# geobacter-rs/rav1e

Measured on AMD Instinct MI355X. Metric: encoded frames/sec + Mpixels/sec, 4K 8-bit speed=10, 1/2/4/8 GPU vs host CPU, higher is better.
Workload: dtype u8

## Files before the change

rav1e_amd/csrc/rv_quant.h:

```cpp
#pragma once

#include "rv_device.h"
#include "rv_quant_tables.h"
#include "rv_rate_table.h"

namespace rv {

struct QCtx {
  int log_tx_scale;
  int32_t dc_quant, dc_offset, ac_quant, ac_offset0, ac_offset1, deadzone;
  uint32_t dc_a, dc_b, dc_s, ac_a, ac_b, ac_s;
};

__host__ __device__ __forceinline__ int q_log_tx_scale(int area) {
  return (area > 256) + (area > 1024);
}

__device__ __forceinline__ int q_lookup(int ac, int qindex, int delta_q, int bd) {
  int i = qindex + delta_q;
  i = i < 0 ? 0 : i > 255 ? 255 : i;
  return RV_QLOOKUP[(3 * ac + (bd - 8) / 2) * 256 + i];
}

__device__ __forceinline__ void q_divu_gen(uint32_t d, uint32_t &a, uint32_t &b, uint32_t &s) {
// ... 98 lines not shown
      q = q_divu(wadd(v, q_signum(v) * c.dc_offset), c.dc_a, c.dc_b, c.dc_s);
    } else if (i <= eob) {
      const int32_t a = v < 0 ? -v : v;
      const int32_t o = v > 0 && a >= (mode ? acq : acq2) ? c.ac_offset1 : c.ac_offset0;
      q = q_divu(wadd(v, q_signum(v) * o), c.ac_a, c.ac_b, c.ac_s);
      mode = (mode != 0 && q == 0) ? 0 : (q > 1 ? 1 : mode);
    } else {
      q = 0;
    }
    const int32_t r = wadd(wmul(q, i == 0 ? c.dc_quant : c.ac_quant), (q >> 31) & roff) >> s;
    put(scan[i], q, r);
  }
  return eob;
}

__device__ __forceinline__ int32_t q_dequant(const QCtx &c, int32_t q, int i) {
  return wadd(wmul(q, i == 0 ? c.dc_quant : c.ac_quant), (q >> 31) & ((1 << c.log_tx_scale) - 1)) >>
         c.log_tx_scale;
}

__device__ __forceinline__ uint64_t q_estimate_rate(int qindex, int tx_size, uint64_t fd) {
  const uint32_t *row =
      RV_RDO_RATE_TABLE + ((qindex / RV_RDO_QUANT_DIV) * 19 + tx_size) * RV_RDO_NUM_BINS;
  uint64_t down = fd / RV_RATE_EST_BIN_SIZE;
  down = down < RV_RDO_NUM_BINS - 2 ? down : RV_RDO_NUM_BINS - 2;
  const uint64_t up = down + 1;
  const int64_t x0 = (int64_t)(down * RV_RATE_EST_BIN_SIZE);
  const int64_t y0 = row[down], y1 = row[up];
  const int64_t slope = (int64_t)((uint64_t)(y1 - y0) << 8) / RV_RATE_EST_BIN_SIZE;
  const int64_t r = y0 + ((int64_t)((uint64_t)((int64_t)fd - x0) * (uint64_t)slope) >> 8);
// ... 5 lines not shown
```

rav1e_amd/csrc/rv_rdo.h:

```cpp
#pragma once

#include "rv_chain.h"
#include "rv_device.h"
#include "rv_quant.h"

namespace rv {

struct RdoPlane {
  rv_plane org;
  rv_plane ref[2];
  rv_plane dst;
  int32_t *levels;
  uint64_t *out;
  QCtx q;
};

struct RdoWinner {
  int32_t c;
  int32_t skip;
  double cost;
  uint64_t dist;
};

struct RdoArgs {
// ... 25 lines not shown

int rv_quant_ctx(int qindex, int tx_area, int is_intra, int bit_depth, int dc_delta_q,
                 int ac_delta_q, rv::QCtx *out);

int rv_rdo_candidates(const rv::RdoArgs &luma, const rv::RdoArgs &chroma, int hbd,
                      hipStream_t s, bool compound = false);

int rv_rdo_blocks2(const rv::RdoArgs &l, const rv::RdoArgs &c, int nl, int nc, int hbd,
                   hipStream_t s, int mode);
int rv_rdo_blocks(const rv::RdoArgs &a, bool luma, int nplanes, int n_tx_size, int hbd,
                  hipStream_t s, int mode);

int rv_rdo_args_put(const rv::RdoArgs *h, int n, rv::RdoArgs *dev, hipStream_t s);
int rv_rdo_candidates_list(const rv::RdoArgs *h, const rv::RdoArgs *dev, int nsets, int mode_a,
                           int hbd, hipStream_t s, int max_grid = 0, uint32_t *kp_cnt = nullptr,
                           unsigned long long *kp_t = nullptr);

int rv_rdo_intra(const rv::RdoArgs &luma, const rv::RdoArgs &chroma, int hbd, hipStream_t s);
```

rav1e_amd/csrc/rv_rdo.hip:

```cpp
#include <stdio.h>
#include <stdlib.h>
#include <string.h>

#include <type_traits>

#include "rv_intra.h"
#include "rv_rdo.h"
#include "rv_tx.h"

namespace rv {


__constant__ int8_t kRdoReg[2][16][8] = {
    {{0, 0, 0, 127, 0, 0, 0, 0}, {0, 2, -6, 126, 8, -2, 0, 0},
     {0, 2, -10, 122, 18, -4, 0, 0}, {0, 2, -12, 116, 28, -8, 2, 0},
     {0, 2, -14, 110, 38, -10, 2, 0}, {0, 2, -14, 102, 48, -12, 2, 0},
     {0, 2, -16, 94, 58, -12, 2, 0}, {0, 2, -14, 84, 66, -12, 2, 0},
     {0, 2, -14, 76, 76, -14, 2, 0}, {0, 2, -12, 66, 84, -14, 2, 0},
     {0, 2, -12, 58, 94, -16, 2, 0}, {0, 2, -12, 48, 102, -14, 2, 0},
     {0, 2, -10, 38, 110, -14, 2, 0}, {0, 2, -8, 28, 116, -12, 2, 0},
     {0, 0, -4, 18, 122, -10, 2, 0}, {0, 0, -2, 8, 126, -6, 2, 0}},
    {{0, 0, 0, 127, 0, 0, 0, 0}, {0, 0, -4, 126, 8, -2, 0, 0},
     {0, 0, -8, 122, 18, -4, 0, 0}, {0, 0, -10, 116, 28, -6, 0, 0},
     {0, 0, -12, 110, 38, -8, 0, 0}, {0, 0, -12, 102, 48, -10, 0, 0},
// ... 248 lines not shown
#pragma unroll 1
    for (int r0 = 0; r0 < RB; r0 += U) {
#pragma unroll
      for (int u = 0; u < U; u++) {
        const int r = r0 + u;
        g0[(u + 6) & 7] = mc_h<Px>(f0, w0 + (r + 6) * (P / 4), col, ib);
        g1[(u + 6) & 7] = mc_h<Px>(f1, w1 + (r + 6) * (P / 4), col, ib);
        const int32_t t = mc_prep_v(f0, g0, u, ib) + mc_prep_v(f1, g1, u, ib);
        pred[(band * RB + r) * N + col] = (Px)clamp_med3(round_shift(t, ib + 1), 0, maxv);
      }
    }
  }
  wave_sync();
}

__device__ __forceinline__ double rdo_bias(const RdoArgs &a, int mi_x, int mi_y, int m = 2) {
  if (!a.imp) return 0.65;
  const int x2 = mi_x + m < a.w_in_b ? mi_x + m : a.w_in_b;
  const int y2 = mi_y + m < a.h_in_b ? mi_y + m : a.h_in_b;
  float tot = 0.f;
  for (int y = mi_y; y < y2; y++)
    for (int x = mi_x; x < x2; x++) tot = __fadd_rn(tot, a.imp[(y >> 1) * a.w_imp + (x >> 1)]);
  return (double)__fdiv_rn(__fdiv_rn(tot, (float)(m * m)), 3.0f) + 0.65;
}
__device__ __forceinline__ uint64_t rdo_biased(uint64_t v, double bias) {
  return (uint64_t)((double)v * bias);
}

__device__ __forceinline__ uint64_t rdo_cdef_finish(int32_t ss, int32_t sd, uint32_t ss2,
                                                    uint32_t sd2, uint32_t ssd, int bd);
// ... 347 lines not shown
#pragma unroll 8
    for (int i = lane; i < N * DPR; i += LPB) {
      const int r = i / DPR, c = (i - r * DPR) * PPD;
      uint32_t v;
      __builtin_memcpy(&v, pred + r * N + c, 4);
      if (valid) __builtin_memcpy(dp + r * ds + c * B, &v, 4);
    }
    return;
  }
  const uint64_t d = group_sum<LPB>(rdo_dist_biased<Px, N, LPB, LUMA>(a, jb, o, ost, pred));
  if (valid && lane == 0) pl.out[(int64_t)jb.oi * 3 + 1] = d;
}

__host__ __device__ constexpr int cmax(int a, int b) { return a > b ? a : b; }

template <typename Px, typename Mid, int NPART>
struct LumaLds {
  static constexpr int kWinP = sizeof(Px) == 1 ? 80 : 144;
  static constexpr int kWinRows = 64 / NPART + 7;
  static constexpr int kCompRows = sizeof(Px) == 1 ? 16 : 8;
  static constexpr int kScr =
      cmax(cmax(cmax(kWinRows * kWinP, 16 * 65 * 4), 32 * 66 * (int)sizeof(Mid)),
           2 * (kCompRows + 7) * kWinP);
  static constexpr int kSlot = (kScr + 64 * 64 * (int)sizeof(Px) + 15) / 16 * 16;
};


template <typename Px>
__device__ __forceinline__ uint64_t luma_dist(const RdoArgs &a, const RdoJob &j, const Px *o,
                                              int64_t os, const Px *pred) {
  const int lane = rv_tid() & 63, by = lane >> 3, bx = lane & 7;
  const uint64_t v =
      rdo_cdef_8x8<Px>(o + (int64_t)(by * 8) * os + bx * 8, os, pred + by * 8 * 64 + bx * 8, 64, a.bd);
  const int px = j.bx + bx * 8, py = j.by + by * 8;
  return group_sum<64>(rdo_biased(v, rdo_bias(a, px >> 2, py >> 2)));
}

template <typename Px, int NPART, int MODE>
__device__ __forceinline__ void luma_front(const RdoArgs &a, const RdoPlane &pl, int t,
                                           const RdoJob &jb, bool valid, uint8_t *scr, Px *pred,
                                           bool skip_dist = true) {
  constexpr int N = 64, B = (int)sizeof(Px);
  constexpr int P = LumaLds<Px, int16_t, NPART>::kWinP;
  constexpr int RP = N / NPART;
  static_assert(RP % 8 == 0, "MC rows run in groups of 8");
  const int lane = rv_tid() & 63;
  const rv_plane &ref = pl.ref[jb.ref];
  const int ox = 0, oy = 0;
  const int bd = a.bd, ib = bd == 12 ? 2 : 4, maxv = (1 << bd) - 1;

  if constexpr (MODE == 3) {
    intra_fill<Px, 64, 64>(jb, reinterpret_cast<int32_t *>(scr), pred, bd, lane);
  } else if (MODE == 1 || (MODE == 2 && jb.comp)) {
    mc_compound<Px, 64, LumaLds<Px, int16_t, NPART>::kCompRows>(
        a, pl, jb, reinterpret_cast<uint32_t *>(scr), pred);
  } else
  {
    uint32_t *win = reinterpret_cast<uint32_t *>(scr);
// ... 79 lines not shown
          if (rf) {
            int32_t s = 0;
#pragma unroll
            for (int k = 1; k < 7; k++) s += __mul24(yt[k], ring[(u + k) & 7]);
            v = round_shift(s, vshift);
          } else {
            v = cf ? round_shift(ring[(u + 3) & 7], ib) : ring[(u + 3) & 7];
          }
          pred[(RP * half + r) * N + col] = (Px)clamp_med3(v, 0, maxv);
        }
      }
    }
    wave_sync();
  }

  const Px *o = plane_ptr<Px>(pl.org, jb.bx, jb.by);
  if (!a.commit && skip_dist) {
    const uint64_t d = luma_dist<Px>(a, jb, o, pl.org.stride, pred);
    if (valid && lane == 0) pl.out[(int64_t)jb.oi * 3 + 0] = d;
  }
  int s0, s1, s2;
  fwd_shifts<N>((bd - 8) / 2, s0, s1, s2);
  int32_t *fmid = reinterpret_cast<int32_t *>(scr);
  {
    int32_t v[N];
#pragma unroll
    for (int r = 0; r < N; r++) {
      const int16_t d = (int16_t)((int16_t)o[(int64_t)r * pl.org.stride + lane] -
                                  (int16_t)pred[r * N + lane]);
      v[r] = rdo_rsa((int32_t)d, -s0);
    }
    tx::fwd1d<1, N>(v, v);
#pragma unroll
    for (int r = 0; r < 16; r++) fmid[r * 65 + lane] = rdo_rsa(v[r], -s1);
  }
// ... 46 lines not shown
  const int32_t *src = fmid + (rr >> 1) * 65 + (rr & 1) * 32;
#pragma unroll
  for (int c = 0; c < 32; c++) {
    const int32_t x = src[c];
    if (pk) pk[c] = x;
    v[c] = tx::clampv(x, range);
  }
#pragma unroll
  for (int c = 32; c < 64; c++) v[c] = 0;
}
template <typename Mid>
__device__ __forceinline__ void luma_inv_row_tx(int32_t *v, Mid *dst, int range, int crange) {
  tx::inv1d<1, 64>(v, range);
#pragma unroll
  for (int c = 0; c < 64; c++) dst[c] = (Mid)tx::clampv(round_shift(v[c], 2), crange);
}

template <typename Px, typename Mid>
__device__ __forceinline__ void luma_back(const RdoArgs &a, const RdoPlane &pl, int t,
                                          const RdoJob &jb, bool valid, const Mid *imid,
                                          Px *pred) {
  constexpr int N = 64, B = (int)sizeof(Px);
  const int lane = rv_tid() & 63;
  const int bd = a.bd, maxv = (1 << bd) - 1;
  const int crange = bd + 6 > 16 ? bd + 6 : 16;
  {
    int32_t v[N];
#pragma unroll
    for (int r = 0; r < N; r++) v[r] = r < 32 ? (int32_t)imid[r * 66 + lane] : 0;
    tx::inv1d<1, N>(v, crange);
// ... 86 lines not shown
  if (b < luma.n_tx && b >= rdo_ntx(luma)) return;
  if (b < luma.n_tx)
    rdo_luma_body<Px, Mid, 2, MODE>(luma, luma.p[0], b, lds,
                              reinterpret_cast<Px *>(lds + L::kScr), scan);
  else
    rdo_chroma_pair<Px, MODE>(chroma, b - luma.n_tx, reinterpret_cast<int32_t *>(lds),
                        reinterpret_cast<Px *>(lds + 2 * 32 * 33 * 4), scan);
}

template <typename Px>
struct QuadLds {
  using L = LumaLds<Px, int16_t, sizeof(Px) == 1 ? 2 : 4>;
  static constexpr int kBytes = cmax(4 * L::kSlot, 3 * kChromaPair(sizeof(Px)));
};

#ifndef RV_RDO_PHASES
#define RV_RDO_PHASES 0
#endif
__device__ unsigned long long g_rdo_ph[3][8];
struct QuadPh {
  unsigned long long t[5];
};

template <typename Px, int MODE>
__device__ __forceinline__ void rdo_quad_luma(const RdoArgs &luma, int b, int n, int var,
                                              uint8_t *lds, const uint16_t *scan,
                                              QuadPh *ph = nullptr) {
  using L = typename QuadLds<Px>::L;
  constexpr int NPART = sizeof(Px) == 1 ? 2 : 4;
  const int wave = __builtin_amdgcn_readfirstlane(rv_tid() >> 6), lane = rv_tid() & 63;
  auto slot = [&](int q) __attribute__((always_inline)) { return lds + q * L::kSlot; };
  auto fmid = [&](int q) __attribute__((always_inline)) {
    return reinterpret_cast<int32_t *>(slot(q));
  };
  auto imid = [&](int q) __attribute__((always_inline)) {
    return reinterpret_cast<int16_t *>(slot(q));
  };
  auto pred = [&](int q) __attribute__((always_inline)) {
    return reinterpret_cast<Px *>(slot(q) + L::kScr);
  };
  const int t0 = 4 * b, t = t0 + wave;
  if (t0 >= n) return;
  const bool valid = t < n;
  RdoJob jb;
  if constexpr (MODE == 3)
    jb = rdo_job_intra<Px, 64>(luma, 0, valid ? t : n - 1);
  else
    jb = rdo_job<64>(luma, luma.p[0], valid ? t : n - 1);
  const bool late_dist = (var & 1) && !luma.commit;
  const bool prio = (var & 2) != 0;
  if (valid)
    luma_front<Px, NPART, MODE>(luma, luma.p[0], t, jb, true, slot(wave), pred(wave), !late_dist);
  __syncthreads();
  if (RV_RDO_PHASES && ph) ph->t[1] = wall_clock64();
  if (wave == 0) {
    if (prio) __builtin_amdgcn_s_setprio(2);
    const int q = lane >> 4;
    if (t0 + q < n) luma_fwd_row(fmid(q) + (lane & 15) * 65, luma.bd);
    if (prio) __builtin_amdgcn_s_setprio(0);
  } else if (late_dist && valid) {
    const uint64_t d = luma_dist<Px>(luma, jb, plane_ptr<Px>(luma.p[0].org, jb.bx, jb.by),
                                     luma.p[0].org.stride, pred(wave));
    if (lane == 0) luma.p[0].out[(int64_t)jb.oi * 3 + 0] = d;
  }
  __syncthreads();
  if (RV_RDO_PHASES && ph) ph->t[2] = wall_clock64();
  if (valid) luma_quantize(luma, luma.p[0], t, jb, true, fmid(wave), scan);
// ... 12 lines not shown
  } else if (wave == 2 && late_dist) {
    RdoJob j0;
    if constexpr (MODE == 3)
      j0 = rdo_job_intra<Px, 64>(luma, 0, t0);
    else
      j0 = rdo_job<64>(luma, luma.p[0], t0);
    const uint64_t d = luma_dist<Px>(luma, j0, plane_ptr<Px>(luma.p[0].org, j0.bx, j0.by),
                                     luma.p[0].org.stride, pred(0));
    if (lane == 0) luma.p[0].out[(int64_t)j0.oi * 3 + 0] = d;
  }
  __syncthreads();
  if (RV_RDO_PHASES && ph) ph->t[4] = wall_clock64();
  if (valid) luma_back<Px, int16_t>(luma, luma.p[0], t, jb, true, imid(wave), pred(wave));
}

template <typename Px, int MODE>
__device__ __forceinline__ void rdo_quad_chroma(const RdoArgs &chroma, int c, int pairs,
                                                uint8_t *lds, const uint16_t *scan) {
  const int wave = __builtin_amdgcn_readfirstlane(rv_tid() >> 6);
  const int pair = 3 * c + wave;
  if (wave == 3 || pair >= 2 * pairs) return;
  uint8_t *w = lds + wave * kChromaPair(sizeof(Px));
  rdo_chroma_pair<Px, MODE>(chroma, pair, reinterpret_cast<int32_t *>(w),
                            reinterpret_cast<Px *>(w + 2 * 32 * 33 * 4), scan, pairs);
}

template <typename Px, int MODE>
__device__ __forceinline__ void rdo_quad_chroma4(const RdoArgs &chroma, int c, int n, uint8_t *lds,
                                                 const uint16_t *scan) {
  constexpr int kSlab = rdo_slab_bytes<Px, 32>();
// ... 43 lines not shown
  __shared__ uint16_t scan[1024];
  if (kp_t && threadIdx.x == 0) atomicMin(kp_t, (unsigned long long)wall_clock64());
  const RdoArgs &la = A[0], &ca = A[1], &lb = A[2], &cb = A[3];
  const int na = rdo_ntx(la), ma = rdo_ntx(ca);
  const int nb = nsets > 1 ? rdo_ntx(lb) : 0, mb = nsets > 1 ? rdo_ntx(cb) : 0;
  if (kp_cnt && blockIdx.x == 0 && threadIdx.x == 0) {
    atomicAdd(kp_cnt + (MA ? 1 : 0), (uint32_t)na);
    atomicAdd(kp_cnt + (MA ? 3 : 2), (uint32_t)ma);
    if (nsets > 1) {
      atomicAdd(kp_cnt + (MB ? 1 : 0), (uint32_t)nb);
      atomicAdd(kp_cnt + (MB ? 3 : 2), (uint32_t)mb);
    }
  }
  const int pa = (ma + 1) / 2, pb = (mb + 1) / 2;
  const bool c4 = (var & 32) != 0;
  const int e0 = (na + 3) / 4, e1 = e0 + (c4 ? (2 * ma + 3) / 4 : (2 * pa + 2) / 3);
  const int e2 = e1 + (nb + 3) / 4, e3 = e2 + (c4 ? (2 * mb + 3) / 4 : (2 * pb + 2) / 3);
  const bool phd = RV_RDO_PHASES && (var & 16) && rv_tid() == 0;
  for (int b = blockIdx.x; b < e3; b += gridDim.x) {
    QuadPh ph;
    ph.t[0] = phd ? wall_clock64() : 0;
    QuadPh *pp = phd ? &ph : nullptr;
    int set = 2;
    if (b < e0) {
      stage_scan(scan, la.q_tx_index);
      rdo_quad_luma<Px, MA>(la, b, na, var, lds, scan, pp);
      set = MA;
    } else if (b < e1) {
      stage_scan(scan, ca.q_tx_index);
      if (c4)
        rdo_quad_chroma4<Px, MA>(ca, b - e0, ma, lds, scan);
      else
        rdo_quad_chroma<Px, MA>(ca, b - e0, pa, lds, scan);
    } else if (b < e2) {
      stage_scan(scan, lb.q_tx_index);
      rdo_quad_luma<Px, MB>(lb, b - e1, nb, var, lds, scan, pp);
      set = MB;
    } else {
      stage_scan(scan, cb.q_tx_index);
      if (c4)
        rdo_quad_chroma4<Px, MB>(cb, b - e2, mb, lds, scan);
      else
        rdo_quad_chroma<Px, MB>(cb, b - e2, pb, lds, scan);
    }
    __syncthreads();
    if (phd) {
      const unsigned long long te = wall_clock64();
      if (set < 2) {
        for (int k = 0; k < 4; k++) atomicAdd(&g_rdo_ph[set][k], ph.t[k + 1] - ph.t[k]);
        atomicAdd(&g_rdo_ph[set][4], te - ph.t[4]);
      } else {
        atomicAdd(&g_rdo_ph[2][0], te - ph.t[0]);
      }
      atomicAdd(&g_rdo_ph[set][5], 1ull);
    }
  }
  if (kp_t && threadIdx.x == 0) atomicMax(kp_t + 1, (unsigned long long)wall_clock64());
}

__global__ __launch_bounds__(256) void rdo_args_store_kernel(RdoArgs a0, RdoArgs a1, RdoArgs a2,
                                                              RdoArgs a3, int n, RdoArgs *out) {
  static_assert(sizeof(RdoArgs) % 4 == 0, "word copy");
  constexpr int W = (int)(sizeof(RdoArgs) / 4);
  for (int i = threadIdx.x; i < n * W; i += blockDim.x) {
    const int k = i / W, w = i - k * W;
// ... 129 lines not shown
  else
    rdo_launch<0>(luma, chroma, hbd, s, cpairs);
  RV_HIP_CHECK_LAUNCH();
  return RV_OK;
}

int rv_rdo_args_put(const RdoArgs *h, int n, RdoArgs *dev, hipStream_t s) {
  if (!h || !dev || n < 1 || n > 4) return rv_set_error(RV_EINVAL, "rv_rdo_args_put: bad arguments");
  rdo_args_store_kernel<<<1, 256, 0, s>>>(h[0], h[n > 1 ? 1 : 0], h[n > 2 ? 2 : 0], h[n > 3 ? 3 : 0],
                                          n, dev);
  RV_HIP_CHECK_LAUNCH();
  return RV_OK;
}

int rv_rdo_candidates_list(const RdoArgs *h, const RdoArgs *dev, int nsets, int mode_a, int hbd,
                           hipStream_t s, int max_grid, uint32_t *kp_cnt, unsigned long long *kp_t) {
  if (!h || !dev || nsets < 1 || nsets > 2 || mode_a < 0 || mode_a > 1 || (nsets == 2 && mode_a) ||
      h[0].commit || h[0].bd == 12)
    return rv_set_error(RV_EINVAL, "rv_rdo_candidates_list: bad arguments");
  for (int k = 0; k < 2 * nsets; k++)
    if (!h[k].list || !h[k].count)
      return rv_set_error(RV_EINVAL, "rv_rdo_candidates_list: the sets must be list-driven");
  static const bool phases = getenv("RAV1E_HIP_RDO_PHASES") && getenv("RAV1E_HIP_RDO_PHASES")[0] == '1';
  const int var = kRdoVariant | (phases && max_grid > 0 ? 16 : 0) | (max_grid > 0 ? 32 : 0);
  unsigned full = 0;
  for (int k = 0; k < nsets; k++)
    full += (unsigned)((h[2 * k].n_tx + 3) / 4) +
            ((var & 32) ? (unsigned)(2 * h[2 * k + 1].n_tx + 3) / 4
                        : (unsigned)(2 * ((h[2 * k + 1].n_tx + 1) / 2) + 2) / 3);
  unsigned grid = std::min(full, kF4Pool);
  if (max_grid > 0) grid = std::min(grid, (unsigned)max_grid);
  if (grid == 0) return RV_OK;
#define RV_LIST(PX, MA, MB) \
  rdo_quad_list_kernel<PX, MA, MB><<<grid, 256, 0, s>>>(dev, nsets, var, kp_cnt, kp_t)
  if (hbd) {
    if (nsets == 2) RV_LIST(uint16_t, 0, 1); else if (mode_a) RV_LIST(uint16_t, 1, 1); else RV_LIST(uint16_t, 0, 0);
  } else {
    if (nsets == 2) RV_LIST(uint8_t, 0, 1); else if (mode_a) RV_LIST(uint8_t, 1, 1); else RV_LIST(uint8_t, 0, 0);
  }
#undef RV_LIST
  RV_HIP_CHECK_LAUNCH();
  return RV_OK;
// ... 26 lines not shown
    else if (n_tx_size == 16) rdo_small_launch<16, true>(a, nplanes, hbd, s, mode);
    else if (n_tx_size == 8) rdo_small_launch<8, true>(a, nplanes, hbd, s, mode);
    else return rv_set_error(RV_EINVAL, "rv_rdo_blocks: luma size");
  } else {
    if (n_tx_size == 32) rdo_small_launch<32, false>(a, nplanes, hbd, s, mode);
    else if (n_tx_size == 16) rdo_small_launch<16, false>(a, nplanes, hbd, s, mode);
    else if (n_tx_size == 8) rdo_small_launch<8, false>(a, nplanes, hbd, s, mode);
    else if (n_tx_size == 4) rdo_small_launch<4, false>(a, nplanes, hbd, s, mode);
    else return rv_set_error(RV_EINVAL, "rv_rdo_blocks: chroma size");
  }
  RV_HIP_CHECK_LAUNCH();
  return RV_OK;
}

extern "C" int rv_rdo_phase_dump(void) {
  unsigned long long h[3][8];
  if (hipDeviceSynchronize() != hipSuccess || hipMemcpyFromSymbol(h, HIP_SYMBOL(g_rdo_ph), sizeof(h)) != hipSuccess)
    return rv_set_error(RV_EHIP, "rv_rdo_phase_dump");
  const double us = 0.01;
  static const char *kName[2] = {"single", "compound"};
  for (int m = 0; m < 2; m++) {
    const double n = h[m][5] ? (double)h[m][5] : 1.0;
    fprintf(stderr,
            "[f4 phases] %s luma quads %llu: front %.2f, row DCT %.2f, quantize %.2f, inverse rows %.2f, "
            "back %.2f us per quad\n",
            kName[m], h[m][5], h[m][0] * us / n, h[m][1] * us / n, h[m][2] * us / n, h[m][3] * us / n,
            h[m][4] * us / n);
  }
  fprintf(stderr, "[f4 phases] chroma triples %llu: %.2f us each\n", h[2][5],
          h[2][0] * us / (h[2][5] ? (double)h[2][5] : 1.0));
  memset(h, 0, sizeof(h));
  return hipMemcpyToSymbol(HIP_SYMBOL(g_rdo_ph), h, sizeof(h)) == hipSuccess ? RV_OK
                                                                           : rv_set_error(RV_EHIP, "rv_rdo_phase_dump");
}
```

rav1e_amd/csrc/rv_replay.hip:

```cpp
#include <string.h>

#include <chrono>
#include <condition_variable>
#include <algorithm>
#include <deque>
#include <mutex>
#include <thread>
#include <vector>

#include "rv_chain.h"
#include "rv_device.h"
#include "rv_ec.h"
#include "rv_intra.h"
#include "rv_intra_pass.h"
#include "rv_mvref.h"
#include "rv_impwin.h"
#include "rv_lrf.h"
#include "rv_rdo.h"
#include <string>

#if __has_include(<rccl/rccl.h>)
#include <rccl/rccl.h>
#define RV_HAVE_RCCL 1
#else
// ... 46 lines not shown
int rv_cdef_filter_frame_dev(const rv_plane src[3], const rv_plane dst[3], int width, int height,
                             const uint8_t *d_skip, int mi_stride, const uint8_t *d_dir,
                             const int32_t *d_var, const uint8_t *d_cdef_index,
                             const uint8_t *y_strengths, const uint8_t *uv_strengths, int damping,
                             int bit_depth, hipStream_t s);
int rv_plane_pyramid(const rv_plane *y, const rv_plane *h, const rv_plane *q, void *stream);
int rv_synth_frame(const rv_plane *y, const rv_plane *u, const rv_plane *v, int t, int bit_depth,
                   void *stream);

namespace rv {

constexpr int kSb = 64;
constexpr int kSlots = 24;
constexpr int kWordsPerRef = 2 + 8 + 2 + 2 + 32 + 8;
constexpr int kRoundGrid = 256;
constexpr int kMaxGroups = 8;

struct Geo {
  int W, H, xdec, ydec, bd, hbd;
  int w_in_b, h_in_b;
  int tx0, ty0, tw, th;
  int tws, ths;
  int nsb, R, M, C;
  int cw, ch;
  int w_imp, h_imp;
  int vis_w, vis_h;
};

__host__ __device__ inline int div_trunc8(int v) { return v / 8; }

// ... 3184 lines not shown
    RV_EV(8);
    score_wave_kernel<<<(g.nsb + 3) / 4, 256, 0, st>>>(
        g, cg, L.lambda, L.ds[1], L.ds[2], r->sub, r->l_out, r->c_out, r->c_out + nct * 3, ntx_c,
        r->win, r->coarse, r->half, r->full, r->look, r->half_l, r->words, r->cand_count,
        r->tail + 2, r->cand_evals + 2 * slot * kLevels, r->leaf_count, nullptr, nullptr,
        r->exact ? r->dec_lv[lv] : nullptr, 0);
    return RV_OK;
  };
  uint32_t q_first = 0;
  auto f3_f4_list = [&](hipStream_t xs, uint32_t q) -> int {
    const int32_t *acnt = slot_cnt(q);
    int lg = q == q_first ? nr * g.R : 0;
    const int hint = q == q_first ? -1 : r->rr.last_count;
    const int hsb = hint >= 0 ? std::max(2 * hint, 16) : 0;
    int f4_grid = 0;
    if (hsb) {
      lg = std::min(hsb * g.R, 512);
      f4_grid = std::min(6 * hsb, 1024);
    }
    RV_R(kp_open(xs));
    RV_R(rv_diamond_f2_f3(&cur.hres, refs_h, r->jobs_half[lv], r->half, ma.f2dirty, &cur.y,
                          refs_y, r->jobs_full[lv], r->full, ma.f3dirty, &to_sub, g.R, nr, g.bd,
                          mvl(q), acnt, lg, xs, r->jobs_sub[lv], r->sub, kp_acc, kp_ts()));
    RV_R(kp_close(xs));
    const int rg = hsb ? std::min(kRoundGrid, std::max((14 * hsb + 255) / 256, (hsb + 3) / 4))
                       : kRoundGrid;
    round_lists_kernel<<<rg, 256, 0, xs>>>(
        cg, r->sub, nsingle, r->cand_list, r->cand_count, mvl(q), acnt,
        CandKeys{r->cand_key, (uint32_t)(r->coded + 1), 1});
    if (f4_list) {
      RV_R(kp_open(xs, 1));
      RV_R(rv_rdo_candidates_list(f4h, r->f4_args, cg.comp ? 2 : 1, 0, g.hbd, xs, f4_grid, kp_f4,
                                  kp_ts(1)));
      RV_R(kp_close(xs, 1));
    } else {
      RV_R(rv_rdo_candidates(la4, ca4, g.hbd, xs));
      if (cg.comp) RV_R(rv_rdo_candidates(lc4, cc4, g.hbd, xs, true));
    }
    score_wave_kernel<<<rg, 256, 0, xs>>>(
        g, cg, L.lambda, L.ds[1], L.ds[2], r->sub, r->l_out, r->c_out, r->c_out + nct * 3, ntx_c,
        r->win, r->coarse, r->half, r->full, r->look, r->half_l, r->words, r->cand_count, nullptr,
        nullptr, nullptr, mvl(q), acnt, r->dec_lv[lv], 1);
    return RV_OK;
  };
  RV_R(f3_f4());
  const int budget = g.tws + 2 * g.ths - 2;
  int mv_runs = 0;
  auto mv_rounds_run = [&](const uint8_t *iwas, bool *changed) -> int {
// ... 531 lines not shown
```

Before: 177.8.

## Add workgroup-cooperative solo luma RDO path for small list-driven F4 rounds

Adds a 'solo' mode in which a whole 256-thread workgroup processes one 64x64 luma candidate instead of four candidates per workgroup (one per wave). Motion compensation is split into bands across waves, column DCT and skip distortion run concurrently on different waves, and quantization becomes workgroup-wide with cross-wave EOB and mode reduction through LDS. The host enables solo mode when the hinted candidate count is small enough, and raises the grid accordingly. The aim is better latency and occupancy for late rounds with few candidates, at the cost of more __syncthreads barriers and extra phase-timing instrumentation.

```diff
diff --git a/rav1e_amd/csrc/rv_quant.h b/rav1e_amd/csrc/rv_quant.h
--- a/rav1e_amd/csrc/rv_quant.h
+++ b/rav1e_amd/csrc/rv_quant.h
@@ -136,6 +136,82 @@
   return eob;
 }
 
+template <int N, typename Co, typename Put>
+__device__ __forceinline__ int quantize_block_wg(const QCtx &c, const uint16_t *scan, Co co,
+                                                 Put put, int32_t *xw) {
+  constexpr int K = N / 256;
+  static_assert(N % 256 == 0 && K <= 16, "whole chunks, coefficients held in registers");
+  const int wl = rv_tid() & 63, wave = __builtin_amdgcn_readfirstlane(rv_tid() >> 6);
+  const int i0 = (rv_tid() & 255) * K;
+  const int s = c.log_tx_scale;
+  const int32_t acq = c.ac_quant, acq2 = 2 * c.ac_quant;
+  int32_t cf[K];
+#pragma unroll
+  for (int k = 0; k < K; k++) cf[k] = (int32_t)((uint32_t)co(scan[i0 + k]) << s);
+  int last = 0;
+#pragma unroll
+  for (int k = 0; k < K; k++) {
+    const int32_t v = cf[k] >> s;
+    if (i0 + k >= 1 && (v < 0 ? -v : v) >= c.deadzone) last = i0 + k;
+  }
+  const uint64_t sig = __ballot(last >= 1);
+  const int wlast = sig ? __shfl(last, 63 - __builtin_clzll(sig), 64) : 0;
+  if (wl == 0) xw[wave] = wlast;
+  __syncthreads();
+  int eob = 1;
+#pragma unroll
+  for (int w = 0; w < 4; w++) {
+    const int e = xw[w];
+    if (e) eob = e;
+  }
+  int map = 2;
+#pragma unroll
+  for (int k = 0; k < K; k++) {
+    const int i = i0 + k;
+    if (i >= 1 && i <= eob) {
+      const int32_t v = cf[k], a = v < 0 ? -v : v;
+      const int32_t o0 = v > 0 && a >= acq2 ? c.ac_offset1 : c.ac_offset0;
+      const int32_t o1 = v > 0 && a >= acq ? c.ac_offset1 : c.ac_offset0;
+      const int t0 = v > 0 && a + o0 >= acq2;
+      const int t1 = a + o1 >= acq;
+      const int f0 = map & 1, f1 = (map >> 1) & 1;
+      map = (f0 ? t1 : t0) | ((f1 ? t1 : t0) << 1);
+    }
+  }
+  const uint64_t nonid = __ballot(map != 2);
+  const uint64_t ones = __ballot(map == 3);
+  if (wl == 0) xw[4 + wave] = nonid ? (int)((ones >> (63 - __builtin_clzll(nonid))) & 1) : 2;
+  __syncthreads();
+  int mode = 1;
+#pragma unroll
+  for (int w = 0; w < 3; w++) {
+    const int m = xw[4 + w];
+    if (w < wave && m != 2) mode = m;
+  }
+  const uint64_t below = nonid & ((1ull << wl) - 1);
+  if (below) mode = (int)((ones >> (63 - __builtin_clzll(below))) & 1);
+  const int32_t roff = (1 << s) - 1;
+#pragma unroll
+  for (int k = 0; k < K; k++) {
+    const int i = i0 + k;
+    const int32_t v = cf[k];
+    int32_t q;
+    if (i == 0) {
+      q = q_divu(wadd(v, q_signum(v) * c.dc_offset), c.dc_a, c.dc_b, c.dc_s);
+    } else if (i <= eob) {
+      const int32_t a = v < 0 ? -v : v;
+      const int32_t o = v > 0 && a >= (mode ? acq : acq2) ? c.ac_offset1 : c.ac_offset0;
+      q = q_divu(wadd(v, q_signum(v) * o), c.ac_a, c.ac_b, c.ac_s);
+      mode = (mode != 0 && q == 0) ? 0 : (q > 1 ? 1 : mode);
+    } else {
+      q = 0;
+    }
+    const int32_t r = wadd(wmul(q, i == 0 ? c.dc_quant : c.ac_quant), (q >> 31) & roff) >> s;
+    put(scan[i], q, r);
+  }
+  return eob;
+}
+
 __device__ __forceinline__ int32_t q_dequant(const QCtx &c, int32_t q, int i) {
   return wadd(wmul(q, i == 0 ? c.dc_quant : c.ac_quant), (q >> 31) & ((1 << c.log_tx_scale) - 1)) >>
          c.log_tx_scale;
diff --git a/rav1e_amd/csrc/rv_rdo.h b/rav1e_amd/csrc/rv_rdo.h
--- a/rav1e_amd/csrc/rv_rdo.h
+++ b/rav1e_amd/csrc/rv_rdo.h
@@ -63,6 +63,6 @@
 int rv_rdo_args_put(const rv::RdoArgs *h, int n, rv::RdoArgs *dev, hipStream_t s);
 int rv_rdo_candidates_list(const rv::RdoArgs *h, const rv::RdoArgs *dev, int nsets, int mode_a,
                            int hbd, hipStream_t s, int max_grid = 0, uint32_t *kp_cnt = nullptr,
-                           unsigned long long *kp_t = nullptr);
+                           unsigned long long *kp_t = nullptr, bool solo = false);
 
 int rv_rdo_intra(const rv::RdoArgs &luma, const rv::RdoArgs &chroma, int hbd, hipStream_t s);
diff --git a/rav1e_amd/csrc/rv_rdo.hip b/rav1e_amd/csrc/rv_rdo.hip
--- a/rav1e_amd/csrc/rv_rdo.hip
+++ b/rav1e_amd/csrc/rv_rdo.hip
@@ -286,6 +286,59 @@
   wave_sync();
 }
 
+template <typename Px, int N, int RB>
+__device__ __forceinline__ void mc_compound_bands(const RdoArgs &a, const RdoPlane &pl,
+                                                  const RdoJob &jb, uint32_t *win, Px *pred,
+                                                  int band0, int nb) {
+  constexpr int B = (int)sizeof(Px);
+  constexpr int P = B == 1 ? ((N + 8 + 15) / 16) * 16 : ((2 * (N + 8) + 15) / 16) * 16;
+  constexpr int kRowDw = ((N + 7) * B + 3) / 4, kTot = (RB + 7) * kRowDw;
+  static_assert((RB % 8 == 0 || RB < 8) && N % RB == 0, "bands of whole 8-row groups");
+  constexpr int U = RB < 8 ? RB : 8;
+  const int col = rv_tid() & (N - 1);
+  const int ib = a.bd == 12 ? 2 : 4, maxv = (1 << a.bd) - 1;
+  const McF f0 = mc_setup<Px>(jb.cf, jb.rf, a.mb_w, a.mb_h);
+  const McF f1 = mc_setup<Px>(jb.cf2, jb.rf2, a.mb_w, a.mb_h);
+  uint32_t *w0 = win, *w1 = win + (RB + 7) * (P / 4);
+  const uint8_t *sp0 = (const uint8_t *)plane_ptr<Px>(pl.ref[0], jb.src_x + jb.ox - 3, jb.src_y + jb.oy - 3);
+  const uint8_t *sp1 =
+      (const uint8_t *)plane_ptr<Px>(pl.ref[1], jb.src2_x + jb.ox - 3, jb.src2_y + jb.oy - 3);
+  const int64_t rs0 = (int64_t)pl.ref[0].stride * B, rs1 = (int64_t)pl.ref[1].stride * B;
+#pragma unroll 1
+  for (int band = band0; band < band0 + nb; band++) {
+    if (band != band0) wave_sync();
+#pragma unroll 2
+    for (int i = col; i < kTot; i += N) {
+      const int r = i / kRowDw, d = i - r * kRowDw;
+      uint32_t v0, v1;
+      __builtin_memcpy(&v0, sp0 + (band * RB + r) * rs0 + 4 * d, 4);
+      __builtin_memcpy(&v1, sp1 + (band * RB + r) * rs1 + 4 * d, 4);
+      w0[r * (P / 4) + d] = B == 1 ? v0 ^ 0x80808080u : v0;
+      w1[r * (P / 4) + d] = B == 1 ? v1 ^ 0x80808080u : v1;
+    }
+    wave_sync();
+    int32_t g0[8], g1[8];
+#pragma unroll
+    for (int k = 1; k < 6; k++) {
+      g0[k] = mc_h<Px>(f0, w0 + k * (P / 4), col, ib);
+      g1[k] = mc_h<Px>(f1, w1 + k * (P / 4), col, ib);
+    }
+    g0[0] = g0[6] = g0[7] = g1[0] = g1[6] = g1[7] = 0;
+#pragma unroll 1
+    for (int r0 = 0; r0 < RB; r0 += U) {
+#pragma unroll
+      for (int u = 0; u < U; u++) {
+        const int r = r0 + u;
+        g0[(u + 6) & 7] = mc_h<Px>(f0, w0 + (r + 6) * (P / 4), col, ib);
+        g1[(u + 6) & 7] = mc_h<Px>(f1, w1 + (r + 6) * (P / 4), col, ib);
+        const int32_t t = mc_prep_v(f0, g0, u, ib) + mc_prep_v(f1, g1, u, ib);
+        pred[(band * RB + r) * N + col] = (Px)clamp_med3(round_shift(t, ib + 1), 0, maxv);
+      }
+    }
+  }
+  wave_sync();
+}
+
 __device__ __forceinline__ double rdo_bias(const RdoArgs &a, int mi_x, int mi_y, int m = 2) {
   if (!a.imp) return 0.65;
   const int x2 = mi_x + m < a.w_in_b ? mi_x + m : a.w_in_b;
@@ -663,6 +716,14 @@
 
 __host__ __device__ constexpr int cmax(int a, int b) { return a > b ? a : b; }
 
+#ifndef RV_RDO_PHASES
+#define RV_RDO_PHASES 0
+#endif
+struct QuadPh {
+  unsigned long long t[5];
+  unsigned long long f[3];
+};
+
 template <typename Px, typename Mid, int NPART>
 struct LumaLds {
   static constexpr int kWinP = sizeof(Px) == 1 ? 80 : 144;
@@ -674,7 +735,6 @@
   static constexpr int kSlot = (kScr + 64 * 64 * (int)sizeof(Px) + 15) / 16 * 16;
 };
 
-
 template <typename Px>
 __device__ __forceinline__ uint64_t luma_dist(const RdoArgs &a, const RdoJob &j, const Px *o,
                                               int64_t os, const Px *pred) {
@@ -685,12 +745,181 @@
   return group_sum<64>(rdo_biased(v, rdo_bias(a, px >> 2, py >> 2)));
 }
 
+template <typename Px>
+__device__ __forceinline__ uint64_t luma_dist_rows(const RdoArgs &a, const RdoJob &j, const Px *o,
+                                                   int64_t os, const Px *pred, int part,
+                                                   int nparts) {
+  const int lane = rv_tid() & 63, row = lane >> 3, bx = lane & 7;
+  int32_t kss = 0, ksd = 0;
+  uint32_t kss2 = 0, ksd2 = 0, kssd = 0;
+  int kby = -1, it = 0;
+#pragma unroll 1
+  for (int by = part; by < 8; by += nparts, it++) {
+    const Px *op = o + (int64_t)(by * 8 + row) * os + bx * 8;
+    const Px *dp = pred + (by * 8 + row) * 64 + bx * 8;
+    int32_t ss = 0, sd = 0;
+    uint32_t ss2 = 0, sd2 = 0, ssd = 0;
+#pragma unroll
+    for (int i = 0; i < 8; i++) {
+      const int32_t sv = op[i], e = dp[i];
+      ss += sv;
+      sd += e;
+      ss2 += (uint32_t)wmul24(sv, sv);
+      sd2 += (uint32_t)wmul24(e, e);
+      ssd += (uint32_t)wmul24(sv, e);
+    }
+#pragma unroll
+    for (int m = 8; m < 64; m <<= 1) {
+      ss += __shfl_xor(ss, m, 64);
+      sd += __shfl_xor(sd, m, 64);
+      ss2 += __shfl_xor(ss2, m, 64);
+      sd2 += __shfl_xor(sd2, m, 64);
+      ssd += __shfl_xor(ssd, m, 64);
+    }
+    if (row == it) {
+      kss = ss, ksd = sd, kss2 = ss2, ksd2 = sd2, kssd = ssd;
+      kby = by;
+    }
+  }
+  uint64_t acc = 0;
+  if (kby >= 0) {
+    const uint64_t v = rdo_cdef_finish(kss, ksd, kss2, ksd2, kssd, a.bd);
+    acc = rdo_biased(v, rdo_bias(a, (j.bx + bx * 8) >> 2, (j.by + kby * 8) >> 2));
+  }
+  return group_sum<64>(acc);
+}
+
+template <typename Px, int RP, int P>
+__device__ __forceinline__ void luma_put_bands(const RdoArgs &a, const RdoPlane &pl,
+                                               const RdoJob &jb, uint32_t *win, Px *pred,
+                                               int band0, int nb) {
+  constexpr int N = 64, B = (int)sizeof(Px);
+  static_assert(RP % 8 == 0, "MC rows run in groups of 8");
+  const int lane = rv_tid() & 63;
+  const rv_plane &ref = pl.ref[jb.ref];
+  const int ox = 0, oy = 0;
+  const int bd = a.bd, ib = bd == 12 ? 2 : 4, maxv = (1 << bd) - 1;
+  const int cf = jb.cf, rf = jb.rf;
+  const int8_t *xf = kRdoReg[a.mb_w <= 4][cf];
+  const int8_t *yf = kRdoReg[a.mb_h <= 4][rf];
+  int yt[8];
+#pragma unroll
+  for (int k = 0; k < 8; k++) yt[k] = yf[k];
+  uint32_t xp[4];
+  int xsum = 0;
+  if constexpr (B == 1) {
+#pragma unroll
+    for (int h = 0; h < 2; h++)
+      xp[h] = (uint32_t)(uint8_t)xf[4 * h] | ((uint32_t)(uint8_t)xf[4 * h + 1] << 8) |
+              ((uint32_t)(uint8_t)xf[4 * h + 2] << 16) | ((uint32_t)(uint8_t)xf[4 * h + 3] << 24);
+#pragma unroll
+    for (int k = 0; k < 8; k++) xsum += xf[k];
+    xp[2] = xp[3] = 0;
+  } else {
+#pragma unroll
+    for (int h = 0; h < 3; h++)
+      xp[h] = (uint32_t)(uint16_t)(int16_t)xf[2 * h + 1] |
+              ((uint32_t)(uint16_t)(int16_t)xf[2 * h + 2] << 16);
+    xp[3] = 0;
+  }
+  const int col = lane;
+  auto hval = [&](int tr) __attribute__((always_inline)) -> int32_t {
+    const uint32_t *row = win + tr * (P / 4);
+    if constexpr (B == 1) {
+      const int d0 = col >> 2, sh = col & 3;
+      const uint32_t w0 = row[d0], w1 = row[d0 + 1], w2 = row[d0 + 2];
+      const uint32_t lo = __builtin_amdgcn_alignbyte(w1, w0, sh);
+      const uint32_t hi = __builtin_amdgcn_alignbyte(w2, w1, sh);
+      if (!cf) return (int32_t)((lo >> 24) ^ 0x80u);
+      int32_t s = dot4_i8(lo, xp[0], 128 * xsum);
+      s = dot4_i8(hi, xp[1], s);
+      return (int32_t)(int16_t)round_shift(s, 7 - ib);
+    } else {
+      const int c1 = col + 1, d0 = c1 >> 1, sh = (c1 & 1) * 2;
+      uint32_t w[4];
+#pragma unroll
+      for (int k = 0; k < 4; k++) w[k] = row[d0 + k];
+      uint32_t pp[3];
+#pragma unroll
+      for (int k = 0; k < 3; k++) pp[k] = __builtin_amdgcn_alignbyte(w[k + 1], w[k], sh);
+      if (!cf) return (int32_t)(pp[1] & 0xffffu);
+      int32_t s = 0;
+#pragma unroll
+      for (int k = 0; k < 3; k++)
+        s = dot2_i16(pp[k], xp[k], s);
+      return (int32_t)(int16_t)round_shift(s, 7 - ib);
+    }
+  };
+  const int vshift = cf ? 7 + ib : 7;
+  constexpr int kRowDw = ((N + 7) * B + 3) / 4;
+  constexpr int kTot = (RP + 7) * kRowDw;
+  const int64_t rs = (int64_t)ref.stride * B;
+#pragma unroll 1
+  for (int half = band0; half < band0 + nb; half++) {
+    const uint8_t *sp =
+        (const uint8_t *)plane_ptr<Px>(ref, jb.src_x + ox - 3, jb.src_y + oy - 3 + RP * half);
+    if (half != band0) wave_sync();
+#pragma unroll 4
+    for (int i = lane; i < kTot; i += 64) {
+      const int r = i / kRowDw, d = i - r * kRowDw;
+      uint32_t v;
+      __builtin_memcpy(&v, sp + r * rs + 4 * d, 4);
+      win[r * (P / 4) + d] = B == 1 ? v ^ 0x80808080u : v;
+    }
+    wave_sync();
+    int32_t ring[8];
+#pragma unroll
+    for (int k = 1; k < 6; k++) ring[k] = hval(k);
+    ring[0] = ring[6] = ring[7] = 0;
+#pragma unroll 1
+    for (int r0 = 0; r0 < RP; r0 += 8) {
+#pragma unroll
+      for (int u = 0; u < 8; u++) {
+        const int r = r0 + u;
+        ring[(u + 6) & 7] = hval(r + 6);
+        int32_t v;
+        if (rf) {
+          int32_t s = 0;
+#pragma unroll
+          for (int k = 1; k < 7; k++) s += __mul24(yt[k], ring[(u + k) & 7]);
+          v = round_shift(s, vshift);
+        } else {
+          v = cf ? round_shift(ring[(u + 3) & 7], ib) : ring[(u + 3) & 7];
+        }
+        pred[(RP * half + r) * N + col] = (Px)clamp_med3(v, 0, maxv);
+      }
+    }
+  }
+}
+
+template <typename Px>
+__device__ __forceinline__ void luma_col_dct(const RdoArgs &a, const RdoPlane &pl, const RdoJob &jb,
+                                             uint8_t *scr, const Px *pred) {
+  constexpr int N = 64;
+  const int lane = rv_tid() & 63;
+  const Px *o = plane_ptr<Px>(pl.org, jb.bx, jb.by);
+  int s0, s1, s2;
+  fwd_shifts<N>((a.bd - 8) / 2, s0, s1, s2);
+  int32_t *fmid = reinterpret_cast<int32_t *>(scr);
+  int32_t v[N];
+#pragma unroll
+  for (int r = 0; r < N; r++) {
+    const int16_t d = (int16_t)((int16_t)o[(int64_t)r * pl.org.stride + lane] -
+                                (int16_t)pred[r * N + lane]);
+    v[r] = rdo_rsa((int32_t)d, -s0);
+  }
+  tx::fwd1d<1, N>(v, v);
+#pragma unroll
+  for (int r = 0; r < 16; r++) fmid[r * 65 + lane] = rdo_rsa(v[r], -s1);
+}
+
 template <typename Px, int NPART, int MODE>
 __device__ __forceinline__ void luma_front(const RdoArgs &a, const RdoPlane &pl, int t,
                                            const RdoJob &jb, bool valid, uint8_t *scr, Px *pred,
-                                           bool skip_dist = true) {
+                                           bool skip_dist = true, QuadPh *ph = nullptr) {
   constexpr int N = 64, B = (int)sizeof(Px);
   constexpr int P = LumaLds<Px, int16_t, NPART>::kWinP;
+  if (RV_RDO_PHASES && ph) ph->f[0] = wall_clock64();
   constexpr int RP = N / NPART;
   static_assert(RP % 8 == 0, "MC rows run in groups of 8");
   const int lane = rv_tid() & 63;
@@ -800,11 +1029,13 @@
     wave_sync();
   }
 
+  if (RV_RDO_PHASES && ph) ph->f[1] = wall_clock64();
   const Px *o = plane_ptr<Px>(pl.org, jb.bx, jb.by);
   if (!a.commit && skip_dist) {
     const uint64_t d = luma_dist<Px>(a, jb, o, pl.org.stride, pred);
     if (valid && lane == 0) pl.out[(int64_t)jb.oi * 3 + 0] = d;
   }
+  if (RV_RDO_PHASES && ph) ph->f[2] = wall_clock64();
   int s0, s1, s2;
   fwd_shifts<N>((bd - 8) / 2, s0, s1, s2);
   int32_t *fmid = reinterpret_cast<int32_t *>(scr);
@@ -881,6 +1112,23 @@
   tx::inv1d<1, 64>(v, range);
 #pragma unroll
   for (int c = 0; c < 64; c++) dst[c] = (Mid)tx::clampv(round_shift(v[c], 2), crange);
+}
+
+template <typename Px, typename Mid>
+__device__ __forceinline__ void luma_inv_cols(const RdoArgs &a, const Mid *imid, Px *pred) {
+  constexpr int N = 64;
+  const int lane = rv_tid() & 63;
+  const int bd = a.bd, maxv = (1 << bd) - 1;
+  const int crange = bd + 6 > 16 ? bd + 6 : 16;
+  int32_t v[N];
+#pragma unroll
+  for (int r = 0; r < N; r++) v[r] = r < 32 ? (int32_t)imid[r * 66 + lane] : 0;
+  tx::inv1d<1, N>(v, crange);
+#pragma unroll
+  for (int r = 0; r < N; r++) {
+    Px *q = pred + r * N + lane;
+    *q = (Px)clamp_med3(wadd((int32_t)*q, round_shift(v[r], 4)), 0, maxv);
+  }
 }
 
 template <typename Px, typename Mid>
@@ -997,13 +1245,7 @@
   static constexpr int kBytes = cmax(4 * L::kSlot, 3 * kChromaPair(sizeof(Px)));
 };
 
-#ifndef RV_RDO_PHASES
-#define RV_RDO_PHASES 0
-#endif
-__device__ unsigned long long g_rdo_ph[3][8];
-struct QuadPh {
-  unsigned long long t[5];
-};
+__device__ unsigned long long g_rdo_ph[3][10];
 
 template <typename Px, int MODE>
 __device__ __forceinline__ void rdo_quad_luma(const RdoArgs &luma, int b, int n, int var,
@@ -1033,7 +1275,7 @@
   const bool late_dist = (var & 1) && !luma.commit;
   const bool prio = (var & 2) != 0;
   if (valid)
-    luma_front<Px, NPART, MODE>(luma, luma.p[0], t, jb, true, slot(wave), pred(wave), !late_dist);
+    luma_front<Px, NPART, MODE>(luma, luma.p[0], t, jb, true, slot(wave), pred(wave), !late_dist, ph);
   __syncthreads();
   if (RV_RDO_PHASES && ph) ph->t[1] = wall_clock64();
   if (wave == 0) {
@@ -1076,6 +1318,102 @@
   if (valid) luma_back<Px, int16_t>(luma, luma.p[0], t, jb, true, imid(wave), pred(wave));
 }
 
+template <typename Px>
+struct SoloLds {
+  using L = typename QuadLds<Px>::L;
+  static constexpr int kBand = 16;
+  static constexpr int kWin =
+      cmax((kBand + 7) * L::kWinP, 2 * (L::kCompRows + 7) * L::kWinP);
+  static constexpr int kPred = (cmax(4 * kWin, cmax(16 * 65 * 4, 32 * 66 * 2)) + 15) / 16 * 16;
+  static constexpr int kRed = kPred + 64 * 64 * (int)sizeof(Px);
+  static constexpr int kBytes = kRed + 8 * 8 + 8 * 4;
+  static_assert(kWin % 16 == 0 && kBand % L::kCompRows == 0, "aligned regions, whole bands");
+  static_assert(kBytes < QuadLds<Px>::kBytes, "below the quad's footprint");
+};
+
+template <typename Px, int MODE>
+__device__ __forceinline__ void rdo_solo_luma(const RdoArgs &luma, int t, uint8_t *lds,
+                                              const uint16_t *scan, QuadPh *ph = nullptr) {
+  static_assert(MODE == 0 || MODE == 1, "score launches: single-reference or compound");
+  using S = SoloLds<Px>;
+  const int wave = __builtin_amdgcn_readfirstlane(rv_tid() >> 6), lane = rv_tid() & 63;
+  const int role = (wave - t) & 3;
+  const RdoPlane &pl = luma.p[0];
+  Px *pred = reinterpret_cast<Px *>(lds + S::kPred);
+  uint64_t *red = reinterpret_cast<uint64_t *>(lds + S::kRed);
+  int32_t *xw = reinterpret_cast<int32_t *>(red + 8);
+  int32_t *fmid = reinterpret_cast<int32_t *>(lds);
+  int16_t *imid = reinterpret_cast<int16_t *>(lds);
+  const RdoJob jb = rdo_job<64>(luma, pl, t);
+  const Px *o = plane_ptr<Px>(pl.org, jb.bx, jb.by);
+  const int64_t os = pl.org.stride;
+  if (RV_RDO_PHASES && ph) ph->f[0] = wall_clock64();
+  {
+    uint32_t *win = reinterpret_cast<uint32_t *>(lds + wave * S::kWin);
+    if constexpr (MODE == 1) {
+      constexpr int RB = S::L::kCompRows;
+      mc_compound_bands<Px, 64, RB>(luma, pl, jb, win, pred, wave * (S::kBand / RB), S::kBand / RB);
+    } else {
+      luma_put_bands<Px, S::kBand, S::L::kWinP>(luma, pl, jb, win, pred, wave, 1);
+    }
+  }
+  __syncthreads();
+  if (RV_RDO_PHASES && ph) ph->f[1] = ph->f[2] = wall_clock64();
+  if (role == 0) {
+    luma_col_dct<Px>(luma, pl, jb, lds, pred);
+  } else {
+    const uint64_t d = luma_dist_rows<Px>(luma, jb, o, os, pred, role - 1, 3);
+    if (lane == 0) red[role] = d;
+  }
+  __syncthreads();
+  if (RV_RDO_PHASES && ph) ph->t[1] = wall_clock64();
+  if (role == 0) {
+    if (lane < 16) luma_fwd_row(fmid + lane * 65, luma.bd);
+  } else if (role == 1 && lane == 0) {
+    pl.out[(int64_t)jb.oi * 3 + 0] = red[1] + red[2] + red[3];
+  }
+  __syncthreads();
+  if (RV_RDO_PHASES && ph) ph->t[2] = wall_clock64();
+  {
+    uint64_t txd = 0;
+    quantize_block_wg<1024>(
+        pl.q, scan, [&](int pos) { return fmid[(pos >> 6) * 65 + (pos & 63)]; },
+        [&](int pos, int32_t q, int32_t r) {
+          int32_t *e = fmid + (pos >> 6) * 65 + (pos & 63);
+          const int32_t dd = wsub(*e, r);
+          txd += (uint64_t)(int64_t)wmul(dd, dd);
+          *e = r;
+        },
+        xw);
+    txd = group_sum<64>(txd);
+    if (lane == 0) red[4 + wave] = txd;
+  }
+  __syncthreads();
+  if (RV_RDO_PHASES && ph) ph->t[3] = wall_clock64();
+  if (role == 0) {
+    const int range = luma.bd + 8, crange = luma.bd + 6 > 16 ? luma.bd + 6 : 16;
+    int32_t v[64];
+    if (lane < 32) luma_inv_row_load(fmid, lane, v, range, nullptr);
+    wave_sync();
+    if (lane < 32) luma_inv_row_tx(v, imid + lane * 66, range, crange);
+  } else if (role == 1 && lane == 0) {
+    const uint64_t txd = red[4] + red[5] + red[6] + red[7];
+    const int bits = 2 * (3 - pl.q.log_tx_scale);
+    pl.out[(int64_t)jb.oi * 3 + 2] =
+        q_estimate_rate(luma.qindex, luma.tx_size, (txd + (1ull << (bits - 1))) >> bits);
+  }
+  __syncthreads();
+  if (RV_RDO_PHASES && ph) ph->t[4] = wall_clock64();
+  if (role == 0) luma_inv_cols<Px, int16_t>(luma, imid, pred);
+  __syncthreads();
+  {
+    const uint64_t d = luma_dist_rows<Px>(luma, jb, o, os, pred, wave, 4);
+    if (lane == 0) red[wave] = d;
+  }
+  __syncthreads();
+  if (rv_tid() == 0) pl.out[(int64_t)jb.oi * 3 + 1] = red[0] + red[1] + red[2] + red[3];
+}
+
 template <typename Px, int MODE>
 __device__ __forceinline__ void rdo_quad_chroma(const RdoArgs &chroma, int c, int pairs,
                                                 uint8_t *lds, const uint16_t *scan) {
@@ -1149,8 +1487,9 @@
   }
   const int pa = (ma + 1) / 2, pb = (mb + 1) / 2;
   const bool c4 = (var & 32) != 0;
-  const int e0 = (na + 3) / 4, e1 = e0 + (c4 ? (2 * ma + 3) / 4 : (2 * pa + 2) / 3);
-  const int e2 = e1 + (nb + 3) / 4, e3 = e2 + (c4 ? (2 * mb + 3) / 4 : (2 * pb + 2) / 3);
+  const bool solo = (var & 64) != 0;
+  const int e0 = solo ? na : (na + 3) / 4, e1 = e0 + (c4 ? (2 * ma + 3) / 4 : (2 * pa + 2) / 3);
+  const int e2 = e1 + (solo ? nb : (nb + 3) / 4), e3 = e2 + (c4 ? (2 * mb + 3) / 4 : (2 * pb + 2) / 3);
   const bool phd = RV_RDO_PHASES && (var & 16) && rv_tid() == 0;
   for (int b = blockIdx.x; b < e3; b += gridDim.x) {
     QuadPh ph;
@@ -1159,7 +1498,10 @@
     int set = 2;
     if (b < e0) {
       stage_scan(scan, la.q_tx_index);
-      rdo_quad_luma<Px, MA>(la, b, na, var, lds, scan, pp);
+      if (solo)
+        rdo_solo_luma<Px, MA>(la, b, lds, scan, pp);
+      else
+        rdo_quad_luma<Px, MA>(la, b, na, var, lds, scan, pp);
       set = MA;
     } else if (b < e1) {
       stage_scan(scan, ca.q_tx_index);
@@ -1169,7 +1511,10 @@
         rdo_quad_chroma<Px, MA>(ca, b - e0, pa, lds, scan);
     } else if (b < e2) {
       stage_scan(scan, lb.q_tx_index);
-      rdo_quad_luma<Px, MB>(lb, b - e1, nb, var, lds, scan, pp);
+      if (solo)
+        rdo_solo_luma<Px, MB>(lb, b - e1, lds, scan, pp);
+      else
+        rdo_quad_luma<Px, MB>(lb, b - e1, nb, var, lds, scan, pp);
       set = MB;
     } else {
       stage_scan(scan, cb.q_tx_index);
@@ -1184,6 +1529,9 @@
       if (set < 2) {
         for (int k = 0; k < 4; k++) atomicAdd(&g_rdo_ph[set][k], ph.t[k + 1] - ph.t[k]);
         atomicAdd(&g_rdo_ph[set][4], te - ph.t[4]);
+        atomicAdd(&g_rdo_ph[set][6], ph.f[1] - ph.f[0]);
+        atomicAdd(&g_rdo_ph[set][7], ph.f[2] - ph.f[1]);
+        atomicAdd(&g_rdo_ph[set][8], ph.t[1] - ph.f[2]);
       } else {
         atomicAdd(&g_rdo_ph[2][0], te - ph.t[0]);
       }
@@ -1343,7 +1691,8 @@
 }
 
 int rv_rdo_candidates_list(const RdoArgs *h, const RdoArgs *dev, int nsets, int mode_a, int hbd,
-                           hipStream_t s, int max_grid, uint32_t *kp_cnt, unsigned long long *kp_t) {
+                           hipStream_t s, int max_grid, uint32_t *kp_cnt, unsigned long long *kp_t,
+                           bool solo) {
   if (!h || !dev || nsets < 1 || nsets > 2 || mode_a < 0 || mode_a > 1 || (nsets == 2 && mode_a) ||
       h[0].commit || h[0].bd == 12)
     return rv_set_error(RV_EINVAL, "rv_rdo_candidates_list: bad arguments");
@@ -1351,10 +1700,11 @@
     if (!h[k].list || !h[k].count)
       return rv_set_error(RV_EINVAL, "rv_rdo_candidates_list: the sets must be list-driven");
   static const bool phases = getenv("RAV1E_HIP_RDO_PHASES") && getenv("RAV1E_HIP_RDO_PHASES")[0] == '1';
-  const int var = kRdoVariant | (phases && max_grid > 0 ? 16 : 0) | (max_grid > 0 ? 32 : 0);
+  const int var = kRdoVariant | (phases && max_grid > 0 ? 16 : 0) | (max_grid > 0 ? 32 : 0) |
+                  (solo ? 64 : 0);
   unsigned full = 0;
   for (int k = 0; k < nsets; k++)
-    full += (unsigned)((h[2 * k].n_tx + 3) / 4) +
+    full += (unsigned)((var & 64) ? h[2 * k].n_tx : (h[2 * k].n_tx + 3) / 4) +
             ((var & 32) ? (unsigned)(2 * h[2 * k + 1].n_tx + 3) / 4
                         : (unsigned)(2 * ((h[2 * k + 1].n_tx + 1) / 2) + 2) / 3);
   unsigned grid = std::min(full, kF4Pool);
@@ -1411,7 +1761,7 @@
 }
 
 extern "C" int rv_rdo_phase_dump(void) {
-  unsigned long long h[3][8];
+  unsigned long long h[3][10];
   if (hipDeviceSynchronize() != hipSuccess || hipMemcpyFromSymbol(h, HIP_SYMBOL(g_rdo_ph), sizeof(h)) != hipSuccess)
     return rv_set_error(RV_EHIP, "rv_rdo_phase_dump");
   const double us = 0.01;
@@ -1419,10 +1769,10 @@
   for (int m = 0; m < 2; m++) {
     const double n = h[m][5] ? (double)h[m][5] : 1.0;
     fprintf(stderr,
-            "[f4 phases] %s luma quads %llu: front %.2f, row DCT %.2f, quantize %.2f, inverse rows %.2f, "
-            "back %.2f us per quad\n",
-            kName[m], h[m][5], h[m][0] * us / n, h[m][1] * us / n, h[m][2] * us / n, h[m][3] * us / n,
-            h[m][4] * us / n);
+            "[f4 phases] %s luma items %llu: front %.2f (MC %.2f, skip distortion %.2f, residual + "
+            "column DCT %.2f), row DCT %.2f, quantize %.2f, inverse rows %.2f, back %.2f us per item\n",
+            kName[m], h[m][5], h[m][0] * us / n, h[m][6] * us / n, h[m][7] * us / n, h[m][8] * us / n,
+            h[m][1] * us / n, h[m][2] * us / n, h[m][3] * us / n, h[m][4] * us / n);
   }
   fprintf(stderr, "[f4 phases] chroma triples %llu: %.2f us each\n", h[2][5],
           h[2][0] * us / (h[2][5] ? (double)h[2][5] : 1.0));
diff --git a/rav1e_amd/csrc/rv_replay.hip b/rav1e_amd/csrc/rv_replay.hip
--- a/rav1e_amd/csrc/rv_replay.hip
+++ b/rav1e_amd/csrc/rv_replay.hip
@@ -84,6 +84,7 @@
 constexpr int kSlots = 24;
 constexpr int kWordsPerRef = 2 + 8 + 2 + 2 + 32 + 8;
 constexpr int kRoundGrid = 256;
+constexpr int kF4SoloPool = 1024;
 constexpr int kMaxGroups = 8;
 
 struct Geo {
@@ -3298,9 +3299,10 @@
     const int hint = q == q_first ? -1 : r->rr.last_count;
     const int hsb = hint >= 0 ? std::max(2 * hint, 16) : 0;
     int f4_grid = 0;
+    const bool f4_solo = hsb > 0 && 11 * hsb <= kF4SoloPool;
     if (hsb) {
       lg = std::min(hsb * g.R, 512);
-      f4_grid = std::min(6 * hsb, 1024);
+      f4_grid = std::min((f4_solo ? 11 : 6) * hsb, 1024);
     }
     RV_R(kp_open(xs));
     RV_R(rv_diamond_f2_f3(&cur.hres, refs_h, r->jobs_half[lv], r->half, ma.f2dirty, &cur.y,
@@ -3315,7 +3317,7 @@
     if (f4_list) {
       RV_R(kp_open(xs, 1));
       RV_R(rv_rdo_candidates_list(f4h, r->f4_args, cg.comp ? 2 : 1, 0, g.hbd, xs, f4_grid, kp_f4,
-                                  kp_ts(1)));
+                                  kp_ts(1), f4_solo));
       RV_R(kp_close(xs, 1));
     } else {
       RV_R(rv_rdo_candidates(la4, ca4, g.hbd, xs));
```

Measured after the change: 179.1 (median of 6 runs). About the same (+0.7%).
